# thunlp/ConvDR

Measured on AMD Instinct MI355X. Metric: passages encoded/sec + query x passage IP-scored/sec, 768-d, higher is better.
Workload: dtype bf16

## Files before the change

### convdr_amd/csrc/gemm_ln.hpp

```cpp
#pragma once
#include "gemm_nt.hpp"

namespace convdr {

using TileLN = TileCfg<4, 2, 6, 2>;
constexpr int LN_SLICE = 32;
constexpr int LN_R_BYTES = TileLN::TR * 64, LN_L_BYTES = TileLN::TL * 64;
constexpr int LN_SMEM_BYTES = 3 * LN_R_BYTES + 2 * LN_L_BYTES;

struct GemmLnArgs {
  const bf16_t* W;
  const bf16_t* A;
  int64_t rows;
  int K;
  const float* bias;
  const bf16_t* R;
  const float *gamma, *beta;
  float eps;
  bf16_t* X;
  unsigned long long* trace;
  const bf16_t* Wks;
  int a_blocked;
  int dbg_skip_epi;
};
#ifdef CONVDR_ENABLE_TRACE
#define CONVDR_LN_TRACE(ph) \
  if (a.trace && threadIdx.x == 0) a.trace[(size_t)blockIdx.x * 16 + (ph)] = __builtin_amdgcn_s_memtime();
#else
#define CONVDR_LN_TRACE(ph)
#endif

constexpr int LN_DMA_WAVES = 8, LN_DMA_FIRST = 0;
constexpr int LN_W_WAVES = 4, LN_W_FIRST = 0;
constexpr int LN_A_WAVES = 4, LN_A_FIRST = 4;
constexpr int LN_A_AUX = 2;

template <int WAVES = LN_DMA_WAVES, int FIRST = LN_DMA_FIRST>
__device__ __forceinline__ StageSrc ln_stage_src(const bf16_t* __restrict__ G, int64_t ld, int64_t row0, int64_t nrows,
                                                  int wave, int lane) {
  StageSrc s;
  wave = wave >= FIRST ? wave - FIRST : 0;
  int64_t bytes = (nrows - row0) * ld * 2;
  bytes = bytes < 0 ? 0 : (bytes > 0xffffffffll ? 0xffffffffll : bytes);
  const uint64_t base = (uint64_t)(G + row0 * ld);
  const uint32_t lo = __builtin_amdgcn_readfirstlane((uint32_t)base);
  const uint32_t hi = __builtin_amdgcn_readfirstlane((uint32_t)(base >> 32));
  const uint32_t nb = __builtin_amdgcn_readfirstlane((uint32_t)bytes);
  s.rsrc = __builtin_amdgcn_make_buffer_rsrc((void*)(((uint64_t)hi << 32) | lo), 0, nb, 0x00020000);
  const int row = wave * 16 + (lane >> 2);
  const int gch = (lane & 3) ^ ((row >> 2) & 3);
  s.voff = (uint32_t)(row * ld * 2) + gch * 16;
  s.round_pitch = __builtin_amdgcn_readfirstlane((uint32_t)(16 * WAVES * ld * 2));
  return s;
}

template <int ROWS, int WAVES = LN_DMA_WAVES, int FIRST = LN_DMA_FIRST, int AUX = 0>
__device__ __forceinline__ void ln_stage32(const StageSrc& s, int ks, char* lds_tile, int wave,
                                           uint32_t slice_stride = LN_SLICE * 2) {
  if (wave < FIRST || wave >= FIRST + WAVES) return;
  wave -= FIRST;
  constexpr int ROUNDS = ROWS / (16 * WAVES);
  static_assert(ROUNDS * 16 * WAVES == ROWS, "rows must be a multiple of 16 x issuing waves");
#pragma unroll
  for (int i = 0; i < ROUNDS; ++i)
    __builtin_amdgcn_raw_ptr_buffer_load_lds(s.rsrc, (lptr_t)(lds_tile + (i * WAVES + wave) * 16 * 64), 16, s.voff,
                                             i * s.round_pitch + ks * slice_stride, 0, AUX);
}

__global__ void __launch_bounds__(512, 2) k_gemm_resid_ln(const GemmLnArgs a) {
  using T = TileLN;
  extern __shared__ __attribute__((aligned(16))) char smem[];
  const WavePos<T> w;
  const int64_t t0 = (int64_t)blockIdx.x * T::TL;
  char* sW = smem;
  char* sA = smem + 3 * LN_R_BYTES;
  GemmAcc<T> acc;
  acc.zero();
  CONVDR_LN_TRACE(0)
  const int nk = a.K / LN_SLICE;
  const int sw = (w.li >> 2) & 3;
  const int offR = (w.wr * T::MT * 32 + w.li) * 64;
  const int offL = (w.wl * T::NT * 32 + w.li) * 64;

  StageSrc srcW = a.Wks ? ln_stage_src<LN_W_WAVES, LN_W_FIRST>(a.Wks, LN_SLICE, 0, (int64_t)T::TR * (a.K / LN_SLICE), w.wave, w.lane)
                        : ln_stage_src<LN_W_WAVES, LN_W_FIRST>(a.W, a.K, 0, T::TR, w.wave, w.lane);
  const uint32_t w_slice_stride = a.Wks ? T::TR * LN_SLICE * 2 : LN_SLICE * 2;
  StageSrc srcA = ln_stage_src<LN_A_WAVES, LN_A_FIRST>(a.A, a.K, t0, a.rows, w.wave, w.lane);
  uint32_t a_slice_stride = LN_SLICE * 2;
  if (a.a_blocked) {
    const int64_t rows32 = (a.rows + 31) & ~(int64_t)31;
    const int64_t blk_elems = (int64_t)(a.K >> 3) * 256;
    int64_t bytes = (rows32 - t0) / 32 * blk_elems * 2;
    bytes = bytes < 0 ? 0 : (bytes > 0xffffffffll ? 0xffffffffll : bytes);
    const uint64_t base = (uint64_t)(a.A + (t0 >> 5) * blk_elems);
    const uint32_t lo = __builtin_amdgcn_readfirstlane((uint32_t)base);
    const uint32_t hi = __builtin_amdgcn_readfirstlane((uint32_t)(base >> 32));
    const uint32_t nb = __builtin_amdgcn_readfirstlane((uint32_t)bytes);
    srcA.rsrc = __builtin_amdgcn_make_buffer_rsrc((void*)(((uint64_t)hi << 32) | lo), 0, nb, 0x00020000);
    const int wv = w.wave >= LN_A_FIRST ? w.wave - LN_A_FIRST : 0;
    const int row = wv * 16 + (w.lane >> 2);
    const int gch = (w.lane & 3) ^ ((row >> 2) & 3);
    srcA.voff = (uint32_t)((row >> 5) * blk_elems * 2 + gch * 512 + (row & 31) * 16);
    srcA.round_pitch = __builtin_amdgcn_readfirstlane((uint32_t)((16 * LN_A_WAVES / 32) * blk_elems * 2));
    a_slice_stride = 4 * 512;
  }
  static_assert((16 * LN_A_WAVES) % 32 == 0 && TileLN::TL % (16 * LN_A_WAVES) == 0, "blocked A staging: rounds of whole 32-token blocks");
  constexpr int LN_W_DPW = T::TR / (16 * LN_W_WAVES);
  const bool w_wave = w.wave >= LN_W_FIRST && w.wave < LN_W_FIRST + LN_W_WAVES;
  ln_stage32<T::TR, LN_W_WAVES, LN_W_FIRST>(srcW, 0, sW, w.wave, w_slice_stride);
  ln_stage32<T::TL, LN_A_WAVES, LN_A_FIRST, LN_A_AUX>(srcA, 0, sA, w.wave, a_slice_stride);
  if (nk > 1) ln_stage32<T::TR, LN_W_WAVES, LN_W_FIRST>(srcW, 1, sW + LN_R_BYTES, w.wave, w_slice_stride);
#ifdef CONVDR_ENABLE_TRACE
#define CONVDR_LN_STEP(i)                                                                                     \
  if (a.trace && kt == 8 + (i) / 5 && w.lane == 0 && blockIdx.x < 256)                                        \
    a.trace[2048 * 16 + blockIdx.x * 64 + w.wave * 8 + (i)] = __builtin_amdgcn_s_memtime();
#else
#define CONVDR_LN_STEP(i)
#endif
  int wslot = 0;
  for (int kt = 0; kt < nk; ++kt) {
    CONVDR_LN_STEP(5)
    CONVDR_LN_STEP(0)
    if (kt + 1 < nk && w_wave) asm volatile("s_waitcnt vmcnt(%0)" ::"n"(LN_W_DPW) : "memory");
    else lds_dma_wait_all();
    CONVDR_LN_STEP(1)
    lds_barrier();
    CONVDR_LN_STEP(2)
    if (kt + 1 < nk) ln_stage32<T::TL, LN_A_WAVES, LN_A_FIRST, LN_A_AUX>(srcA, kt + 1, sA + ((kt + 1) & 1) * LN_L_BYTES, w.wave, a_slice_stride);
    const bool issue_w = kt + 2 < nk;
    char* w_dst = sW + (wslot == 0 ? 2 : wslot - 1) * LN_R_BYTES;
    CONVDR_LN_STEP(3)
    const char* tR = sW + wslot * LN_R_BYTES + offR;
    const char* tL = sA + (kt & 1) * LN_L_BYTES + offL;
    wslot = wslot == 2 ? 0 : wslot + 1;
    {
      constexpr int UNITS = 2 * T::MT;
      static_assert(T::NT == 2, "TileLN: two activation fragments per sub-step");
      const int ch0 = ((0 + w.hi) ^ sw) * 16, ch1 = ((2 + w.hi) ^ sw) * 16;
      bf16x8 fb[2][T::NT], fa[3];
      auto load_a = [&](int u) { fa[u % 3] = *(const bf16x8*)(tR + (u % T::MT) * 32 * 64 + (u < T::MT ? ch0 : ch1)); };
#pragma unroll
      for (int j = 0; j < T::NT; ++j) fb[0][j] = *(const bf16x8*)(tL + j * 32 * 64 + ch0);
      load_a(0);
      load_a(1);
#pragma unroll
      for (int u = 0; u < UNITS; ++u) {
        if (u + 2 < UNITS) load_a(u + 2);
        if (u == 2) {
#pragma unroll
          for (int j = 0; j < T::NT; ++j) fb[1][j] = *(const bf16x8*)(tL + j * 32 * 64 + ch1);
        }
#pragma unroll
        for (int j = 0; j < T::NT; ++j)
          acc.c[u % T::MT][j] = __builtin_amdgcn_mfma_f32_32x32x16_bf16(fa[u % 3], fb[u / T::MT][j], acc.c[u % T::MT][j], 0, 0, 0);
      }
      __builtin_amdgcn_sched_group_barrier(0x100, T::NT + 2, 0);
#pragma unroll
      for (int u = 0; u < UNITS; ++u) {
        if (u + 2 < UNITS) __builtin_amdgcn_sched_group_barrier(0x100, 1, 0);
        if (u == 2) __builtin_amdgcn_sched_group_barrier(0x100, T::NT, 0);
        __builtin_amdgcn_sched_group_barrier(0x008, T::NT, 0);
      }
    }
    if (issue_w) ln_stage32<T::TR, LN_W_WAVES, LN_W_FIRST>(srcW, kt + 2, w_dst, w.wave, w_slice_stride);
    CONVDR_LN_STEP(4)
  }

  if (a.dbg_skip_epi) {
    float s = 0.f;
#pragma unroll
    for (int mt = 0; mt < T::MT; ++mt)
#pragma unroll
      for (int nt = 0; nt < T::NT; ++nt)
#pragma unroll
        for (int r = 0; r < 16; ++r) s += acc.c[mt][nt][r];
    if (s == 12345.678f) a.X[0] = f32_to_bf16(s);
    return;
  }
  CONVDR_LN_TRACE(1)
  __syncthreads();
  float* sBias = (float*)smem;
  float* sGam = sBias + 768;
  float* sBet = sGam + 768;
  float* sRed = sBet + 768;
  float* sStat = sRed + 128 * 8;
  char* sC = smem + 16384;
  const int slot = w.wr * 2 + w.hi;
  const StageSrc srcR = ln_stage_src(a.R, 768, t0, a.rows, w.wave, w.lane);
  const __amdgpu_buffer_rsrc_t dstX = ln_stage_src(a.X, 768, t0, a.rows, w.wave, w.lane).rsrc;
  typedef __attribute__((address_space(3))) u32x2_t lds_u2_t;
  static_assert((16384 & 511) == 0, "the image base must leave bits 4-8 to the swizzle");
  auto img_base = [&](int lrl) { return lds_off(sC) + (uint32_t)(lrl * 1536 + ((lrl & 31) << 4) + w.hi * 8); };
  auto img_at = [&](uint32_t B, int chunk) {
    return (lds_u2_t*)(uintptr_t)((B ^ (uint32_t)((chunk & 31) << 4)) + (uint32_t)((chunk & ~31) << 4));
  };
  auto opaque = [](int x) {
    asm volatile("" : "+v"(x));
    return x;
  };
  CONVDR_LN_TRACE(2)
#pragma unroll
  for (int nt = 0; nt < T::NT; ++nt) {
    if (nt) __syncthreads();
    const int tid_a = opaque((int)threadIdx.x);
    int lr = tid_a / 96, pp = tid_a - lr * 96;
#pragma unroll
    for (int i = 0; i < 12; ++i) {
      const int c = (pp & ~31) | ((pp ^ lr) & 31);
      const int tok = (lr >> 5) * 64 + nt * 32 + (lr & 31);
      __builtin_amdgcn_raw_ptr_buffer_load_lds(srcR.rsrc, (lptr_t)(sC + (i * 512 + w.wave * 64) * 16), 16,
                                               (uint32_t)(tok * 1536 + c * 16), 0, 0, 0);
      pp += 32; lr += 5;
      if (pp >= 96) { pp -= 96; lr += 1; }
    }
    if (nt == 0) {
      for (int i = threadIdx.x; i < 768; i += 512) { sBias[i] = a.bias[i]; sGam[i] = a.gamma[i]; sBet[i] = a.beta[i]; }
      CONVDR_LN_TRACE(8)
    }
    lds_dma_wait_all();
    if (nt == 0) { CONVDR_LN_TRACE(9) }
    __syncthreads();
    if (nt == 0) { CONVDR_LN_TRACE(10) }
    float s = 0.f;
    const uint32_t imgB = img_base(opaque(w.wl * 32 + w.li));
#pragma unroll
    for (int mt = 0; mt < T::MT; ++mt) {
      u32x2_t res[4];
#pragma unroll
      for (int g = 0; g < 4; ++g) res[g] = *img_at(imgB, (w.wr * T::MT + mt) * 4 + g);
#pragma unroll
      for (int g = 0; g < 4; ++g) {
        f32x16& v = acc.c[mt][nt];
        const float4 bv = *(const float4*)(sBias + w.r_base(mt, g));
        const u32x2_t r = res[g];
        v[4 * g + 0] += bv.x + __uint_as_float(r.x << 16);
        v[4 * g + 1] += bv.y + __uint_as_float(r.x & 0xffff0000u);
        v[4 * g + 2] += bv.z + __uint_as_float(r.y << 16);
        v[4 * g + 3] += bv.w + __uint_as_float(r.y & 0xffff0000u);
        s += (v[4 * g + 0] + v[4 * g + 1]) + (v[4 * g + 2] + v[4 * g + 3]);
      }
    }
    sRed[(w.wl * 64 + nt * 32 + w.li) * 8 + slot] = s;
    if (nt == 0) { CONVDR_LN_TRACE(11) }
  }
  CONVDR_LN_TRACE(3)
  __syncthreads();
  CONVDR_LN_TRACE(4)
  if (threadIdx.x < 128) {
    const float* p = sRed + threadIdx.x * 8;
    sStat[threadIdx.x] = (((p[0] + p[1]) + (p[2] + p[3])) + ((p[4] + p[5]) + (p[6] + p[7]))) * (1.f / 768.f);
  }
  __syncthreads();
  float mean[T::NT];
#pragma unroll
  for (int nt = 0; nt < T::NT; ++nt) {
    mean[nt] = sStat[w.wl * 64 + nt * 32 + w.li];
    float q = 0.f;
#pragma unroll
    for (int mt = 0; mt < T::MT; ++mt)
#pragma unroll
      for (int r = 0; r < 16; ++r) {
        const float d = acc.c[mt][nt][r] - mean[nt];
        q += d * d;
      }
    sRed[(w.wl * 64 + nt * 32 + w.li) * 8 + slot] = q;
  }
  CONVDR_LN_TRACE(5)
  __syncthreads();
  if (threadIdx.x < 128) {
    const float* p = sRed + threadIdx.x * 8;
    const float var = (((p[0] + p[1]) + (p[2] + p[3])) + ((p[4] + p[5]) + (p[6] + p[7]))) * (1.f / 768.f);
    sStat[128 + threadIdx.x] = rsqrtf(var + a.eps);
  }
  __syncthreads();
  CONVDR_LN_TRACE(6)
#pragma unroll
  for (int nt = 0; nt < T::NT; ++nt) {
    if (nt) __syncthreads();
    const float rstd = sStat[128 + w.wl * 64 + nt * 32 + w.li];
    const uint32_t imgB = img_base(opaque(w.wl * 32 + w.li));
#pragma unroll
    for (int mt = 0; mt < T::MT; ++mt)
#pragma unroll
      for (int g = 0; g < 4; ++g) {
        const int f = w.r_base(mt, g);
        const float4 gg = *(const float4*)(sGam + f), bb = *(const float4*)(sBet + f);
        const f32x16& v = acc.c[mt][nt];
        u32x2_t o;
        o.x = pack_bf16x2((v[4 * g + 0] - mean[nt]) * rstd * gg.x + bb.x, (v[4 * g + 1] - mean[nt]) * rstd * gg.y + bb.y);
        o.y = pack_bf16x2((v[4 * g + 2] - mean[nt]) * rstd * gg.z + bb.z, (v[4 * g + 3] - mean[nt]) * rstd * gg.w + bb.w);
        *img_at(imgB, (w.wr * T::MT + mt) * 4 + g) = o;
      }
    if (nt == 0) { CONVDR_LN_TRACE(12) }
    __syncthreads();
    if (nt == 0) { CONVDR_LN_TRACE(13) }
    const int tid_s = opaque((int)threadIdx.x);
    int lr = tid_s / 96, pp = tid_s - lr * 96;
#pragma unroll
    for (int i0 = 0; i0 < 12; i0 += 4) {
      u32x4_t v4[4];
#pragma unroll
      for (int j = 0; j < 4; ++j) v4[j] = *(const u32x4_t*)(sC + ((i0 + j) * 512 + tid_s) * 16);
#pragma unroll
      for (int j = 0; j < 4; ++j) {
        const int c = (pp & ~31) | ((pp ^ lr) & 31);
        const int tok = (lr >> 5) * 64 + nt * 32 + (lr & 31);
        __builtin_amdgcn_raw_buffer_store_b128(v4[j], dstX, (uint32_t)(tok * 1536 + c * 16), 0, NT_LN ? 2 : 0);
        pp += 32; lr += 5;
        if (pp >= 96) { pp -= 96; lr += 1; }
      }
    }
    if (nt == 0) { CONVDR_LN_TRACE(14) }
  }
  CONVDR_LN_TRACE(7)
}

}
```

Baseline: 44930.

## Seed GEMM accumulators with bias and restructure LN epilogue image layout

Initializes the accumulators with the bias vector loaded straight from global memory instead of zeroing them, which removes the bias staging to LDS and the per-element bias add in the epilogue. The residual staging and output stores switch to a banded image layout whose offsets are computed once per thread, replacing the per-iteration div/mod index stepping. Mean subtraction is folded into the variance pass and the sum and variance loops use packed float2 arithmetic (FMA). These changes reduce epilogue ALU and LDS work, at the cost of extra registers live during the GEMM main loop and a more complex address mapping that has to stay consistent between the load and store paths.

Result: no change. 44850 (-0.2%).

```diff
diff --git a/convdr_amd/csrc/gemm_ln.hpp b/convdr_amd/csrc/gemm_ln.hpp
--- a/convdr_amd/csrc/gemm_ln.hpp
+++ b/convdr_amd/csrc/gemm_ln.hpp
@@ -75,7 +75,19 @@
   char* sW = smem;
   char* sA = smem + 3 * LN_R_BYTES;
   GemmAcc<T> acc;
-  acc.zero();
+  auto opaque = [](int x) {
+    asm volatile("" : "+v"(x));
+    return x;
+  };
+  const float* bias_hi = a.bias + 4 * opaque(w.hi);
+#pragma unroll
+  for (int mt = 0; mt < T::MT; ++mt)
+#pragma unroll
+    for (int g = 0; g < 4; ++g) {
+      const float4 bv = *(const float4*)(bias_hi + (w.wr * T::MT + mt) * 32 + 8 * g);
+      acc.c[mt][0][4 * g + 0] = bv.x; acc.c[mt][0][4 * g + 1] = bv.y;
+      acc.c[mt][0][4 * g + 2] = bv.z; acc.c[mt][0][4 * g + 3] = bv.w;
+    }
   CONVDR_LN_TRACE(0)
   const int nk = a.K / LN_SLICE;
   const int sw = (w.li >> 2) & 3;
@@ -107,6 +119,12 @@
   static_assert((16 * LN_A_WAVES) % 32 == 0 && TileLN::TL % (16 * LN_A_WAVES) == 0, "blocked A staging: rounds of whole 32-token blocks");
   constexpr int LN_W_DPW = T::TR / (16 * LN_W_WAVES);
   const bool w_wave = w.wave >= LN_W_FIRST && w.wave < LN_W_FIRST + LN_W_WAVES;
+#pragma unroll
+  for (int mt = 0; mt < T::MT; ++mt) {
+    asm volatile("" : "+v"(acc.c[mt][0]));
+#pragma unroll
+    for (int nt = 1; nt < T::NT; ++nt) acc.c[mt][nt] = acc.c[mt][0];
+  }
   ln_stage32<T::TR, LN_W_WAVES, LN_W_FIRST>(srcW, 0, sW, w.wave, w_slice_stride);
   ln_stage32<T::TL, LN_A_WAVES, LN_A_FIRST, LN_A_AUX>(srcA, 0, sA, w.wave, a_slice_stride);
   if (nk > 1) ln_stage32<T::TR, LN_W_WAVES, LN_W_FIRST>(srcW, 1, sW + LN_R_BYTES, w.wave, w_slice_stride);
@@ -179,8 +197,7 @@
   }
   CONVDR_LN_TRACE(1)
   __syncthreads();
-  float* sBias = (float*)smem;
-  float* sGam = sBias + 768;
+  float* sGam = (float*)smem;
   float* sBet = sGam + 768;
   float* sRed = sBet + 768;
   float* sStat = sRed + 128 * 8;
@@ -190,38 +207,40 @@
   const __amdgpu_buffer_rsrc_t dstX = ln_stage_src(a.X, 768, t0, a.rows, w.wave, w.lane).rsrc;
   typedef __attribute__((address_space(3))) u32x2_t lds_u2_t;
   static_assert((16384 & 511) == 0, "the image base must leave bits 4-8 to the swizzle");
-  auto img_base = [&](int lrl) { return lds_off(sC) + (uint32_t)(lrl * 1536 + ((lrl & 31) << 4) + w.hi * 8); };
+  auto img_base = [&](int lrl) {
+    return lds_off(sC) + (uint32_t)((lrl >> 4) * 24576 + (lrl & 15) * 512 + ((lrl & 31) << 4) + w.hi * 8);
+  };
   auto img_at = [&](uint32_t B, int chunk) {
-    return (lds_u2_t*)(uintptr_t)((B ^ (uint32_t)((chunk & 31) << 4)) + (uint32_t)((chunk & ~31) << 4));
+    return (lds_u2_t*)(uintptr_t)((B ^ (uint32_t)((chunk & 31) << 4)) + (uint32_t)((chunk >> 5) * 8192));
   };
-  auto opaque = [](int x) {
-    asm volatile("" : "+v"(x));
-    return x;
-  };
+  auto img_voff = [](int tid) { return (uint32_t)((tid >> 5) * 1536 + (((tid & 31) ^ (tid >> 5)) << 4)); };
+  auto img_tok0 = [](int rg, int nt) { return (rg >> 1) * 64 + nt * 32 + (rg & 1) * 16; };
+  typedef float f32x2 __attribute__((ext_vector_type(2)));
+  auto pair = [](const f32x16& v, int i) { return f32x2{v[i], v[i + 1]}; };
+  auto set_pair = [](f32x16& v, int i, f32x2 p) { v[i] = p.x; v[i + 1] = p.y; };
   CONVDR_LN_TRACE(2)
 #pragma unroll
   for (int nt = 0; nt < T::NT; ++nt) {
     if (nt) __syncthreads();
     const int tid_a = opaque((int)threadIdx.x);
-    int lr = tid_a / 96, pp = tid_a - lr * 96;
-#pragma unroll
-    for (int i = 0; i < 12; ++i) {
-      const int c = (pp & ~31) | ((pp ^ lr) & 31);
-      const int tok = (lr >> 5) * 64 + nt * 32 + (lr & 31);
-      __builtin_amdgcn_raw_ptr_buffer_load_lds(srcR.rsrc, (lptr_t)(sC + (i * 512 + w.wave * 64) * 16), 16,
-                                               (uint32_t)(tok * 1536 + c * 16), 0, 0, 0);
-      pp += 32; lr += 5;
-      if (pp >= 96) { pp -= 96; lr += 1; }
+    const uint32_t voff_a = img_voff(tid_a);
+#pragma unroll
+    for (int rg = 0; rg < 4; ++rg) {
+      const uint32_t vo = (voff_a ^ (uint32_t)((rg & 1) * 256)) + (uint32_t)(img_tok0(rg, nt) * 1536);
+#pragma unroll
+      for (int band = 0; band < 3; ++band)
+        __builtin_amdgcn_raw_ptr_buffer_load_lds(srcR.rsrc, (lptr_t)(sC + (rg * 3 + band) * 8192 + w.wave * 1024), 16, vo,
+                                                 band * 512, 0, 0);
     }
     if (nt == 0) {
-      for (int i = threadIdx.x; i < 768; i += 512) { sBias[i] = a.bias[i]; sGam[i] = a.gamma[i]; sBet[i] = a.beta[i]; }
+      for (int i = threadIdx.x; i < 768; i += 512) { sGam[i] = a.gamma[i]; sBet[i] = a.beta[i]; }
       CONVDR_LN_TRACE(8)
     }
     lds_dma_wait_all();
     if (nt == 0) { CONVDR_LN_TRACE(9) }
     __syncthreads();
     if (nt == 0) { CONVDR_LN_TRACE(10) }
-    float s = 0.f;
+    f32x2 s2 = {0.f, 0.f};
     const uint32_t imgB = img_base(opaque(w.wl * 32 + w.li));
 #pragma unroll
     for (int mt = 0; mt < T::MT; ++mt) {
@@ -231,16 +250,16 @@
 #pragma unroll
       for (int g = 0; g < 4; ++g) {
         f32x16& v = acc.c[mt][nt];
-        const float4 bv = *(const float4*)(sBias + w.r_base(mt, g));
         const u32x2_t r = res[g];
-        v[4 * g + 0] += bv.x + __uint_as_float(r.x << 16);
-        v[4 * g + 1] += bv.y + __uint_as_float(r.x & 0xffff0000u);
-        v[4 * g + 2] += bv.z + __uint_as_float(r.y << 16);
-        v[4 * g + 3] += bv.w + __uint_as_float(r.y & 0xffff0000u);
-        s += (v[4 * g + 0] + v[4 * g + 1]) + (v[4 * g + 2] + v[4 * g + 3]);
-      }
-    }
-    sRed[(w.wl * 64 + nt * 32 + w.li) * 8 + slot] = s;
+        const f32x2 lo = pair(v, 4 * g) + f32x2{__uint_as_float(r.x << 16), __uint_as_float(r.x & 0xffff0000u)};
+        const f32x2 hi = pair(v, 4 * g + 2) + f32x2{__uint_as_float(r.y << 16), __uint_as_float(r.y & 0xffff0000u)};
+        set_pair(v, 4 * g, lo);
+        set_pair(v, 4 * g + 2, hi);
+        s2 += lo;
+        s2 += hi;
+      }
+    }
+    sRed[(w.wl * 64 + nt * 32 + w.li) * 8 + slot] = s2.x + s2.y;
     if (nt == 0) { CONVDR_LN_TRACE(11) }
   }
   CONVDR_LN_TRACE(3)
@@ -251,19 +270,20 @@
     sStat[threadIdx.x] = (((p[0] + p[1]) + (p[2] + p[3])) + ((p[4] + p[5]) + (p[6] + p[7]))) * (1.f / 768.f);
   }
   __syncthreads();
-  float mean[T::NT];
 #pragma unroll
   for (int nt = 0; nt < T::NT; ++nt) {
-    mean[nt] = sStat[w.wl * 64 + nt * 32 + w.li];
-    float q = 0.f;
+    const float mean = sStat[w.wl * 64 + nt * 32 + w.li];
+    const f32x2 mean2 = {mean, mean};
+    f32x2 q2 = {0.f, 0.f};
 #pragma unroll
     for (int mt = 0; mt < T::MT; ++mt)
 #pragma unroll
-      for (int r = 0; r < 16; ++r) {
-        const float d = acc.c[mt][nt][r] - mean[nt];
-        q += d * d;
-      }
-    sRed[(w.wl * 64 + nt * 32 + w.li) * 8 + slot] = q;
+      for (int r = 0; r < 16; r += 2) {
+        const f32x2 d = pair(acc.c[mt][nt], r) - mean2;
+        set_pair(acc.c[mt][nt], r, d);
+        q2 = __builtin_elementwise_fma(d, d, q2);
+      }
+    sRed[(w.wl * 64 + nt * 32 + w.li) * 8 + slot] = q2.x + q2.y;
   }
   CONVDR_LN_TRACE(5)
   __syncthreads();
@@ -287,27 +307,25 @@
         const float4 gg = *(const float4*)(sGam + f), bb = *(const float4*)(sBet + f);
         const f32x16& v = acc.c[mt][nt];
         u32x2_t o;
-        o.x = pack_bf16x2((v[4 * g + 0] - mean[nt]) * rstd * gg.x + bb.x, (v[4 * g + 1] - mean[nt]) * rstd * gg.y + bb.y);
-        o.y = pack_bf16x2((v[4 * g + 2] - mean[nt]) * rstd * gg.z + bb.z, (v[4 * g + 3] - mean[nt]) * rstd * gg.w + bb.w);
+        o.x = pack_bf16x2(v[4 * g + 0] * rstd * gg.x + bb.x, v[4 * g + 1] * rstd * gg.y + bb.y);
+        o.y = pack_bf16x2(v[4 * g + 2] * rstd * gg.z + bb.z, v[4 * g + 3] * rstd * gg.w + bb.w);
         *img_at(imgB, (w.wr * T::MT + mt) * 4 + g) = o;
       }
     if (nt == 0) { CONVDR_LN_TRACE(12) }
     __syncthreads();
     if (nt == 0) { CONVDR_LN_TRACE(13) }
     const int tid_s = opaque((int)threadIdx.x);
-    int lr = tid_s / 96, pp = tid_s - lr * 96;
+    const uint32_t voff_s = img_voff(tid_s);
 #pragma unroll
     for (int i0 = 0; i0 < 12; i0 += 4) {
       u32x4_t v4[4];
 #pragma unroll
-      for (int j = 0; j < 4; ++j) v4[j] = *(const u32x4_t*)(sC + ((i0 + j) * 512 + tid_s) * 16);
+      for (int j = 0; j < 4; ++j) v4[j] = *(const u32x4_t*)(sC + (i0 + j) * 8192 + tid_s * 16);
 #pragma unroll
       for (int j = 0; j < 4; ++j) {
-        const int c = (pp & ~31) | ((pp ^ lr) & 31);
-        const int tok = (lr >> 5) * 64 + nt * 32 + (lr & 31);
-        __builtin_amdgcn_raw_buffer_store_b128(v4[j], dstX, (uint32_t)(tok * 1536 + c * 16), 0, NT_LN ? 2 : 0);
-        pp += 32; lr += 5;
-        if (pp >= 96) { pp -= 96; lr += 1; }
+        const int rg = (i0 + j) / 3, band = (i0 + j) % 3;
+        __builtin_amdgcn_raw_buffer_store_b128(v4[j], dstX, (voff_s ^ (uint32_t)((rg & 1) * 256)) + (uint32_t)(img_tok0(rg, nt) * 1536),
+                                               band * 512, NT_LN ? 2 : 0);
       }
     }
     if (nt == 0) { CONVDR_LN_TRACE(14) }
```
